# ilur98/DLMC-QUANT

Hardware: AMD Instinct MI355X
Metric: ResNet-50 W8A8 fake-quant fwd images/sec (higher is better)
Workload: dtype i8; 1 GPU; resnet50 W8A8 per-channel fake-quant forward (FSPTQ forms: W minmax_channel s8, A minmax_tensor u8), BN folded first as in FSPTQuant.py:67, fused int8 MFMA conv/linear, frozen execution plan (epilogue-fused ReLU / shortcut / next-layer codes; block end + next 1x1 as one launch; weight codes quantised once at plan build), 2 HIP streams per GPU, 224x224 relu(N(0,1)) pixels, batch 512 per GPU, scales; global_batch=512, parallelism=dp1 (batch-sharded replicas)

## Files before the change

dlmc-quant_amd/csrc/conv_pwr_i8.hip:

```cpp
#include "conv_i8_common.h"

namespace dlmcq {

struct PwrArgs {
  const int8_t* x;
  const int8_t* w;
  const float* s_w;
  const int32_t* wsum;
  const float* bias;
  const float* s_in;
  const float* zp_in;
  const float* residual;
  float* out;
  int f_rowb, f_chunk;
  int M, K, shift, nslice;
  int nblk;
  const int8_t* x2;
  const int8_t* w2;
  const float* s_w2;
  const int32_t* wsum2;
  const float* bias2;
  const float* s_in2;
  const float* zp_in2;
  int shift2, P, Q, H2, W2, stride2;
  FastDiv qdiv, pdiv;
};

constexpr int PWR_BN = 128;
constexpr int PWR_FROW = 36;

__device__ __forceinline__ void bload16s(f32x4& dst, int voff, const v4i& rsrc, int soff) {
  asm volatile("buffer_load_dwordx4 %0, %1, %2, %3 offen" DLMCQ_NT : "=v"(dst) : "v"(voff), "s"(rsrc), "s"(soff) : "memory");
}
__device__ __forceinline__ void bstore16s(const f32x4& v, int voff, const v4i& rsrc, int soff) {
  asm volatile("buffer_store_dwordx4 %0, %1, %2, %3 offen" DLMCQ_NT "\n\ts_nop 1" ::"v"(v), "v"(voff), "s"(rsrc), "s"(soff) : "memory");
}

template <int C, int NW, bool OUTF, bool CODES = true, int C2 = 0, bool SWP = false>
__global__ __launch_bounds__(NW * 64, NW / 4) void conv_pwr_i8_kernel(PwrArgs a, ConvEpi ep) {
  static_assert(OUTF || CODES, "nothing to produce");
  constexpr bool RES = C2 == 0;
  constexpr int NA2 = C2 / 32;
  constexpr int WB2 = C2 * PWR_BN;
  constexpr int NPAR = RES ? 3 : 6;
  constexpr int BN = PWR_BN;
  constexpr int S = C / 64;
  constexpr int NA = C / 32;
  constexpr int NP = BN / 32;
  constexpr int WB = C * BN;
  constexpr int PIECES = S * (BN / 16);
  constexpr int O = OUTF ? 4 : 0;
  constexpr int SROW = BN + 16;
  constexpr int NST = CODES ? 4 : 0;
  extern __shared__ __attribute__((aligned(1024))) int8_t pwr_lds[];
  int8_t* const wl = pwr_lds;
  int8_t* const wl2 = pwr_lds + WB;
  int8_t* const par = pwr_lds + WB + WB2;
  const int tid = threadIdx.x, wave = tid >> 6, lane = tid & 63, l31 = lane & 31, hsel = lane >> 5;
  int8_t* const stg = pwr_lds + WB + WB2 + NPAR * BN * 4 + wave * (32 * SROW + 32 * PWR_FROW * 4);
  float* const fst = reinterpret_cast<float*>(stg + 32 * SROW);
  const int rsel = lane >> 3, q4 = lane & 7;

  const uint32_t b = blockIdx.x;
  const int slice = (int)((b >> 3) % (uint32_t)a.nslice);
  const int group = (int)((b >> 3) / (uint32_t)a.nslice) * 8 + (int)(b & 7u);
  const int ngroups = (int)(gridDim.x / (uint32_t)a.nslice);
  const int n0 = slice * BN;

  {
    const void* arrs[6] = {a.s_w, a.wsum, a.bias, a.s_w2, a.wsum2, a.bias2};
#pragma unroll
    for (int r = 0; r < NPAR; ++r) {
      if (!arrs[r]) {
        for (int c = tid; c < BN; c += NW * 64) reinterpret_cast<float*>(par)[r * BN + c] = 0.0f;
        continue;
      }
      for (int c = wave; c < BN / 64; c += NW)
        __builtin_amdgcn_global_load_lds((gptr_t)(static_cast<const int32_t*>(arrs[r]) + n0 + c * 64 + lane), (lptr_t)(par + (r * BN + c * 64) * 4), 4, 0, 0);
    }
    const int lrow = lane >> 2, pslot = lane & 3;
    for (int pc = wave; pc < PIECES; pc += NW) {
      const int s = pc / (BN / 16), r16 = pc - s * (BN / 16);
      const int row = r16 * 16 + lrow;
      const int d = row & 31;
      const int k = n0 + (row & ~31) + 16 * ((d >> 2) & 1) + 4 * (d >> 3) + (d & 3);
      const int seg = pslot ^ ((row >> 2) & 3);
      __builtin_amdgcn_global_load_lds((gptr_t)(a.w + (int64_t)k * C + s * 64 + seg * 16), (lptr_t)(wl + s * (BN * 64) + r16 * 1024), 16, 0, 0);
    }
    for (int pc = wave; pc < (C2 / 64) * (BN / 16); pc += NW) {
      const int s = pc / (BN / 16), r16 = pc - s * (BN / 16);
      const int row = r16 * 16 + lrow;
      const int d = row & 31;
      const int k = n0 + (row & ~31) + 16 * ((d >> 2) & 1) + 4 * (d >> 3) + (d & 3);
      const int seg = pslot ^ ((row >> 2) & 3);
      __builtin_amdgcn_global_load_lds((gptr_t)(a.w2 + (int64_t)k * C2 + s * 64 + seg * 16), (lptr_t)(wl2 + s * (BN * 64) + r16 * 1024), 16, 0, 0);
    }
  }
  const float zpf = a.zp_in ? a.zp_in[0] : 0.0f;
  const int zpi = (int)__builtin_rintf(zpf);
  const float sin = a.s_in[0];
  const uint32_t xorw = a.shift ? 0x80808080u : 0u;
  const EpiQuant eq(ep, true);
  const v4i r_x = make_rsrc(a.x, (uint32_t)((int64_t)a.M * C));
  const v4i r_c = make_rsrc(CODES ? ep.codes : nullptr, CODES ? (uint32_t)((int64_t)a.M * a.K) : 0u);
  const v4i r_r = make_rsrc(RES ? a.residual : nullptr, RES ? (uint32_t)((int64_t)a.M * a.K * 4) : 0u);
  const v4i r_x2 = make_rsrc(RES ? nullptr : a.x2, RES ? 0u : (uint32_t)((int64_t)(a.M / (a.P * a.Q)) * a.H2 * a.W2 * C2));
  const uint32_t xorw2 = (!RES && a.shift2) ? 0x80808080u : 0u;
  const v4i r_o = make_rsrc(OUTF ? a.out : nullptr, OUTF ? (uint32_t)((int64_t)a.M * a.K * 4) : 0u);
  const int so8 = __builtin_amdgcn_readfirstlane(8 * a.f_rowb);
  const int fchunk = __builtin_amdgcn_readfirstlane(a.f_chunk);
  auto poff = [&](int p) { return (p >> 1) * fchunk + (p & 1) * 128; };

  i32x4 areg[NA];
  i32x4 areg2[RES ? 1 : NA2];
  f32x4 res[2][4];
  auto request = [&](int blk) {
    const int vo = blk < a.nblk ? (blk * 32 + l31) * C + hsel * 16 : BUF_BIG;
    static_for<NA>([&](auto f) { bload16i<decltype(f)::value * 32>(areg[decltype(f)::value], vo, r_x); });
    if constexpr (!RES) {
      const uint32_t m = (uint32_t)(blk * 32 + l31);
      const uint32_t t = fdiv(m, a.qdiv);
      const int q = (int)(m - t * (uint32_t)a.Q);
      const uint32_t n = fdiv(t, a.pdiv);
      const int pp = (int)(t - n * (uint32_t)a.P);
      const int vo2 = blk < a.nblk ? (((int)n * a.H2 + pp * a.stride2) * a.W2 + q * a.stride2) * C2 + hsel * 16 : BUF_BIG;
      static_for<NA2>([&](auto f) { bload16i<(decltype(f)::value % 64) * 32>(areg2[decltype(f)::value], vo2 + (decltype(f)::value / 64) * 2048, r_x2); });
    }
  };
  auto fbase = [&](int blk) { return blk < a.nblk ? (blk * 32 + rsel) * a.f_rowb + slice * 2 * fchunk + 16 * q4 : BUF_BIG; };
  const int stride = ngroups * NW;
  int blk = group * NW + wave;
  request(blk);
  if constexpr (RES) {
    const int vb = fbase(blk);
#pragma unroll
    for (int it = 0; it < 4; ++it) bload16s(res[0][it], vb, r_r, it * so8);
  }
  asm volatile("s_waitcnt vmcnt(0)" ::: "memory");
  __syncthreads();
  if (tid < BN) {
    float* pf = reinterpret_cast<float*>(par) + tid;
    int* pi = reinterpret_cast<int*>(par) + BN + tid;
    *pf = sin * *pf;
    *pi = (a.shift - zpi) * *pi;
    if constexpr (!RES) {
      const float zp2 = a.zp_in2 ? a.zp_in2[0] : 0.0f;
      pf[3 * BN] = a.s_in2[0] * pf[3 * BN];
      pi[3 * BN] = (a.shift2 - (int)__builtin_rintf(zp2)) * pi[3 * BN];
    }
  }
  __syncthreads();

  for (; blk < a.nblk; blk += stride) {
    asm volatile("s_waitcnt vmcnt(%0)" ::"n"(O + NST) : "memory");
#pragma unroll
    for (int f = 0; f < NA; ++f) {
      asm volatile("" : "+v"(areg[f]));
      areg[f] = i32x4{(int)(areg[f].x ^ xorw), (int)(areg[f].y ^ xorw), (int)(areg[f].z ^ xorw), (int)(areg[f].w ^ xorw)};
    }
    if constexpr (!RES) {
#pragma unroll
      for (int f = 0; f < NA2; ++f) {
        asm volatile("" : "+v"(areg2[f]));
        areg2[f] = i32x4{(int)(areg2[f].x ^ xorw2), (int)(areg2[f].y ^ xorw2), (int)(areg2[f].z ^ xorw2), (int)(areg2[f].w ^ xorw2)};
      }
    }
    const int vb = fbase(blk);
    const int vbn = fbase(blk + stride);
    static_for<NP>([&](auto p_c) {
      constexpr int p = decltype(p_c)::value;
      constexpr int cur = p & 1, nxt = cur ^ 1;
      if constexpr (RES) {
#pragma unroll
        for (int it = 0; it < 4; ++it) bload16s(res[nxt][it], (p + 1 < NP ? vb + poff(p + 1) : vbn), r_r, it * so8);
      }
      f32x2 ex[RES ? 1 : 8];
      if constexpr (!RES) {
        i32x16 acc2;
        const i32x4* cop = reinterpret_cast<const i32x4*>(par + (4 * BN + p * 32 + hsel * 16) * 4);
#pragma unroll
        for (int q = 0; q < 4; ++q) {
          const i32x4 c4 = cop[q];
          acc2[4 * q] = c4.x;
          acc2[4 * q + 1] = c4.y;
          acc2[4 * q + 2] = c4.z;
          acc2[4 * q + 3] = c4.w;
        }
        static_for<NA2>([&](auto f_c) {
          constexpr int f = decltype(f_c)::value;
          constexpr int s = f >> 1, ks = f & 1;
          const int sg = ks * 2 + hsel;
          const int brow = p * 32 + l31;
          const i32x4 bf = *reinterpret_cast<const i32x4*>(wl2 + s * (BN * 64) + brow * 64 + ((sg ^ ((brow >> 2) & 3)) << 4));
          acc2 = __builtin_amdgcn_mfma_i32_32x32x32_i8(bf, areg2[f], acc2, 0, 0, 0);
        });
        const int cb2 = p * 32 + hsel * 16;
#pragma unroll
        for (int q = 0; q < 4; ++q) {
          const f32x4 mu = *reinterpret_cast<const f32x4*>(par + (3 * BN + cb2 + 4 * q) * 4);
          const f32x4 bs = *reinterpret_cast<const f32x4*>(par + (5 * BN + cb2 + 4 * q) * 4);
          ex[RES ? 0 : 2 * q] = pk_fma(f32x2{(float)acc2[4 * q], (float)acc2[4 * q + 1]}, f32x2{mu.x, mu.y}, f32x2{bs.x, bs.y});
          ex[RES ? 0 : 2 * q + 1] = pk_fma(f32x2{(float)acc2[4 * q + 2], (float)acc2[4 * q + 3]}, f32x2{mu.z, mu.w}, f32x2{bs.z, bs.w});
        }
      }
      i32x16 acc;
      {
        const i32x4* cop = reinterpret_cast<const i32x4*>(par + (BN + p * 32 + hsel * 16) * 4);
#pragma unroll
        for (int q = 0; q < 4; ++q) {
          const i32x4 c4 = cop[q];
          acc[4 * q] = c4.x;
          acc[4 * q + 1] = c4.y;
          acc[4 * q + 2] = c4.z;
          acc[4 * q + 3] = c4.w;
        }
      }
      static_for<NA>([&](auto f_c) {
        constexpr int f = decltype(f_c)::value;
        constexpr int s = f >> 1, ks = f & 1;
        const int sg = ks * 2 + hsel;
        const int brow = p * 32 + l31;
        const i32x4 bf = *reinterpret_cast<const i32x4*>(wl + s * (BN * 64) + brow * 64 + ((sg ^ ((brow >> 2) & 3)) << 4));
        acc = __builtin_amdgcn_mfma_i32_32x32x32_i8(bf, areg[f], acc, 0, 0, 0);
      });
      if constexpr (p == NP - 1) request(blk + stride);
      const int cb = p * 32 + hsel * 16;
#pragma unroll
      for (int q = 0; q < 4; ++q) {
        const f32x4 mu = *reinterpret_cast<const f32x4*>(par + (cb + 4 * q) * 4);
        const f32x4 bs = *reinterpret_cast<const f32x4*>(par + (2 * BN + cb + 4 * q) * 4);
        f32x2 ya = pk_fma(f32x2{(float)acc[4 * q], (float)acc[4 * q + 1]}, f32x2{mu.x, mu.y}, f32x2{bs.x, bs.y});
        f32x2 yb = pk_fma(f32x2{(float)acc[4 * q + 2], (float)acc[4 * q + 3]}, f32x2{mu.z, mu.w}, f32x2{bs.z, bs.w});
        if constexpr (!RES) {
          ya = SWP ? ex[RES ? 0 : 2 * q] + ya : ya + ex[RES ? 0 : 2 * q];
          yb = SWP ? ex[RES ? 0 : 2 * q + 1] + yb : yb + ex[RES ? 0 : 2 * q + 1];
        }
        *reinterpret_cast<f32x4*>(fst + l31 * PWR_FROW + hsel * 16 + 4 * q) = f32x4{ya.x, ya.y, yb.x, yb.y};
      }
      asm volatile("s_waitcnt lgkmcnt(0)" ::: "memory");
      if constexpr (RES && p > 0) asm volatile("s_waitcnt vmcnt(%0)" ::"n"(O + 4 + (p == NP - 1 ? NA : 0)) : "memory");
      f32x4 v[4];
#pragma unroll
      for (int it = 0; it < 4; ++it) {
        const f32x4 y = *reinterpret_cast<const f32x4*>(fst + (it * 8 + rsel) * PWR_FROW + 4 * q4);
        if constexpr (RES) {
          asm volatile("" : "+v"(res[cur][it]));
          const f32x2 va = f32x2{y.x, y.y} + f32x2{res[cur][it].x, res[cur][it].y};
          const f32x2 vc = f32x2{y.z, y.w} + f32x2{res[cur][it].z, res[cur][it].w};
          v[it] = f32x4{va.x, va.y, vc.x, vc.y};
        } else {
          v[it] = y;
        }
        if constexpr (OUTF) {
          v[it] = relu4_nan(v[it]);
          bstore16s(v[it], vb + poff(p), r_o, it * so8);
        }
      }
      asm volatile("s_waitcnt lgkmcnt(0)" ::: "memory");
      if constexpr (CODES) {
        uint32_t wq[4];
        eq.code4n_plain(v, wq);
#pragma unroll
        for (int it = 0; it < 4; ++it) *reinterpret_cast<uint32_t*>(stg + (it * 8 + rsel) * SROW + p * 32 + 4 * q4) = wq[it];
      }
    });
    if constexpr (CODES) {
      const int vc = blk < a.nblk ? (blk * 32 + rsel) * a.K + n0 + q4 * 16 : BUF_BIG;
#pragma unroll
      for (int it = 0; it < NST; ++it) {
        const i32x4 c16 = *reinterpret_cast<const i32x4*>(stg + (it * 8 + rsel) * SROW + q4 * 16);
        asm volatile("buffer_store_dwordx4 %0, %1, %2, %3 offen\n\ts_nop 1" ::"v"(c16), "v"(vc), "s"(r_c), "s"(it * 8 * a.K) : "memory");
      }
    }
  }
  asm volatile("s_waitcnt vmcnt(0)" ::: "memory");
}

bool conv_pwr_applies(int64_t N, int64_t H, int64_t W, int64_t C, int64_t K, int64_t R, int64_t S, int32_t stride, int32_t pad,
                      int32_t dilation, const ConvEpi& ep, const float* out, const ConvSeg2* seg2) {
  if (R != 1 || S != 1 || pad != 0 || dilation != 1 || !ep.relu || ep.w_off) return false;
  if (ep.relu == DLMCQ_ACT_RELU6) return false;
  if (ep.codes ? !epi_plain(ep) : !out) return false;
  const int64_t P = (H - 1) / stride + 1, Q = (W - 1) / stride + 1;
  const int64_t M = N * P * Q;
  if (seg2) {
    const ConvGeom& g2 = seg2->g;
    if (ep.residual || !out || !ep.codes || g2.R != 1 || g2.S != 1 || g2.pad != 0 || g2.dil != 1 || g2.P != P || g2.Q != Q) return false;
    const bool main_dense = stride == 1 && C == 256 && g2.C == 512, seg_dense = g2.stride == 1 && g2.C == 256 && C == 512;
    if (!main_dense && !seg_dense) return false;
    if ((main_dense ? N * g2.H * g2.W : N * H * W) * 512 >= (int64_t)BUF_BIG) return false;
  } else {
    if (stride != 1 || !ep.residual || !(C == 256 || C == 512)) return false;
    if (M * C >= (int64_t)BUF_BIG) return false;
  }
  if (K % PWR_BN != 0 || K > 4096) return false;
  if (ep.residual && out && ((ep.ctl & DLMCQ_FP32_IN_CHUNK_MAJOR) != 0) != ((ep.ctl & DLMCQ_FP32_OUT_CHUNK_MAJOR) != 0)) return false;
  if ((ep.codes && !aligned16(ep.codes)) || (ep.residual && !aligned16(ep.residual)) || (out && !aligned16(out))) return false;
  if (M < 4096 || M % 32 != 0) return false;
  if (M * K * 4 >= (int64_t)BUF_BIG) return false;
  return true;
}

template <int C, int NW, bool OUTF, bool CODES = true, int C2 = 0, bool SWP = false>
static int pwr_go(const PwrArgs& a0, const ConvEpi& ep, hipStream_t st) {
  constexpr int LDS = (C + C2) * PWR_BN + (C2 ? 6 : 3) * PWR_BN * 4 + NW * (32 * (PWR_BN + 16) + 32 * PWR_FROW * 4);
  static_assert(LDS <= 160 * 1024, "LDS");
  PwrArgs a = a0;
  a.nslice = a.K / PWR_BN;
  static int cus = 0;
  if (!cus) {
    int dev = 0;
    hipDeviceProp_t prop;
    cus = (hipGetDevice(&dev) == hipSuccess && hipGetDeviceProperties(&prop, dev) == hipSuccess && prop.multiProcessorCount > 0)
              ? prop.multiProcessorCount : 256;
  }
  int ngroups = (cus / a.nslice) & ~7;
  if (ngroups < 8) ngroups = 8;
  const int maxg = ((a.nblk + NW - 1) / NW + 7) & ~7;
  if (ngroups > maxg) ngroups = maxg;
  auto kern = conv_pwr_i8_kernel<C, NW, OUTF, CODES, C2, SWP>;
  static bool attr_set = false;
  if (!attr_set) {
    const hipError_t e = hipFuncSetAttribute(reinterpret_cast<const void*>(kern), hipFuncAttributeMaxDynamicSharedMemorySize, LDS);
    if (e != hipSuccess) return (int)e;
    attr_set = true;
  }
  hipLaunchKernelGGL(kern, dim3((uint32_t)(ngroups * a.nslice)), dim3(NW * 64), LDS, st, a, ep);
  return launch_status();
}

int conv_pwr_launch(const int8_t* x, const int8_t* w, float* out, const float* bias, const int32_t* wsum, const float* in_scale,
                    const float* in_zero_point, const float* w_scale, int64_t N, int64_t H, int64_t W, int64_t C, int64_t K, int32_t stride,
                    int shift, const ConvEpi& ep, hipStream_t st, const ConvSeg2* seg2) {
  const int64_t P = (H - 1) / stride + 1, Q = (W - 1) / stride + 1;
  PwrArgs a{};
  a.x = x; a.w = w; a.s_w = w_scale; a.wsum = wsum; a.bias = bias; a.s_in = in_scale; a.zp_in = in_zero_point;
  a.residual = ep.residual; a.out = out;
  a.M = (int)(N * P * Q); a.K = (int)K; a.shift = shift;
  a.nblk = a.M / 32;
  const bool fcm = (ep.ctl & (ep.residual ? DLMCQ_FP32_IN_CHUNK_MAJOR : DLMCQ_FP32_OUT_CHUNK_MAJOR)) != 0;
  a.f_rowb = fcm ? 256 : a.K * 4;
  a.f_chunk = fcm ? a.M * 256 : 256;
#ifndef DLMCQ_PWR_NW256
#define DLMCQ_PWR_NW256 12
#endif
#ifndef DLMCQ_PWR_NW512
#define DLMCQ_PWR_NW512 8
#endif
  constexpr int N2 = DLMCQ_PWR_NW256, N5 = DLMCQ_PWR_NW512;
  if (seg2) {
    const ConvGeom& g2 = seg2->g;
    a.P = (int)P; a.Q = (int)Q;
    a.qdiv = make_fastdiv((uint32_t)Q);
    a.pdiv = make_fastdiv((uint32_t)P);
    if (C == 256) {
      a.x2 = seg2->x; a.w2 = seg2->w; a.s_w2 = seg2->s_w; a.wsum2 = seg2->wsum; a.bias2 = seg2->bias; a.s_in2 = seg2->s_in; a.zp_in2 = seg2->zp_in;
      a.shift2 = seg2->shift; a.H2 = g2.H; a.W2 = g2.W; a.stride2 = g2.stride;
      return pwr_go<256, 6, true, true, 512, false>(a, ep, st);
    }
    a.x = seg2->x; a.w = seg2->w; a.s_w = seg2->s_w; a.wsum = seg2->wsum; a.bias = seg2->bias; a.s_in = seg2->s_in; a.zp_in = seg2->zp_in;
    a.shift = seg2->shift;
    a.x2 = x; a.w2 = w; a.s_w2 = w_scale; a.wsum2 = wsum; a.bias2 = bias; a.s_in2 = in_scale; a.zp_in2 = in_zero_point;
    a.shift2 = shift; a.H2 = (int)H; a.W2 = (int)W; a.stride2 = stride;
    return pwr_go<256, 6, true, true, 512, true>(a, ep, st);
  }
  if (!ep.codes) return C == 256 ? pwr_go<256, N2, true, false>(a, ep, st) : (C == 512 ? pwr_go<512, N5, true, false>(a, ep, st) : DLMCQ_EINVAL);
  if (C == 256) return out ? pwr_go<256, N2, true>(a, ep, st) : pwr_go<256, N2, false>(a, ep, st);
  if (C == 512) return out ? pwr_go<512, N5, true>(a, ep, st) : pwr_go<512, N5, false>(a, ep, st);
  return DLMCQ_EINVAL;
}

}
```

Before: 93720 images/s.

## Extend dual-GEMM projection fusion to the 512/1024-channel stage with 64-wide slices

```diff
diff --git a/dlmc-quant_amd/csrc/conv_pwr_i8.hip b/dlmc-quant_amd/csrc/conv_pwr_i8.hip
--- a/dlmc-quant_amd/csrc/conv_pwr_i8.hip
+++ b/dlmc-quant_amd/csrc/conv_pwr_i8.hip
@@ -36,14 +36,16 @@
   asm volatile("buffer_store_dwordx4 %0, %1, %2, %3 offen" DLMCQ_NT "\n\ts_nop 1" ::"v"(v), "v"(voff), "s"(rsrc), "s"(soff) : "memory");
 }
 
-template <int C, int NW, bool OUTF, bool CODES = true, int C2 = 0, bool SWP = false>
+template <int C, int NW, bool OUTF, bool CODES = true, int C2 = 0, bool SWP = false, int BN = PWR_BN>
 __global__ __launch_bounds__(NW * 64, NW / 4) void conv_pwr_i8_kernel(PwrArgs a, ConvEpi ep) {
   static_assert(OUTF || CODES, "nothing to produce");
+  static_assert(BN == 64 || BN == 128, "slice width");
   constexpr bool RES = C2 == 0;
-  constexpr int NA2 = C2 / 32;
-  constexpr int WB2 = C2 * PWR_BN;
+  constexpr bool DEEP = C2 > 512;
+  static_assert(!DEEP || (BN == 64 && OUTF && CODES && C2 % 64 == 0), "the deep dual form: 64-wide slices, fp32 output and codes");
+  constexpr int NA2 = DEEP ? C2 / 64 : C2 / 32;
+  constexpr int WB2 = C2 * BN;
   constexpr int NPAR = RES ? 3 : 6;
-  constexpr int BN = PWR_BN;
   constexpr int S = C / 64;
   constexpr int NA = C / 32;
   constexpr int NP = BN / 32;
@@ -51,7 +53,9 @@
   constexpr int PIECES = S * (BN / 16);
   constexpr int O = OUTF ? 4 : 0;
   constexpr int SROW = BN + 16;
-  constexpr int NST = CODES ? 4 : 0;
+  constexpr int LPR = BN / 16;
+  constexpr int RPI = 64 / LPR;
+  constexpr int NST = CODES ? 32 / RPI : 0;
   extern __shared__ __attribute__((aligned(1024))) int8_t pwr_lds[];
   int8_t* const wl = pwr_lds;
   int8_t* const wl2 = pwr_lds + WB;
@@ -114,20 +118,36 @@
   i32x4 areg[NA];
   i32x4 areg2[RES ? 1 : NA2];
   f32x4 res[2][4];
-  auto request = [&](int blk) {
+  auto request_main = [&](int blk) {
     const int vo = blk < a.nblk ? (blk * 32 + l31) * C + hsel * 16 : BUF_BIG;
     static_for<NA>([&](auto f) { bload16i<decltype(f)::value * 32>(areg[decltype(f)::value], vo, r_x); });
-    if constexpr (!RES) {
-      const uint32_t m = (uint32_t)(blk * 32 + l31);
-      const uint32_t t = fdiv(m, a.qdiv);
-      const int q = (int)(m - t * (uint32_t)a.Q);
-      const uint32_t n = fdiv(t, a.pdiv);
-      const int pp = (int)(t - n * (uint32_t)a.P);
-      const int vo2 = blk < a.nblk ? (((int)n * a.H2 + pp * a.stride2) * a.W2 + q * a.stride2) * C2 + hsel * 16 : BUF_BIG;
-      static_for<NA2>([&](auto f) { bload16i<(decltype(f)::value % 64) * 32>(areg2[decltype(f)::value], vo2 + (decltype(f)::value / 64) * 2048, r_x2); });
-    }
   };
-  auto fbase = [&](int blk) { return blk < a.nblk ? (blk * 32 + rsel) * a.f_rowb + slice * 2 * fchunk + 16 * q4 : BUF_BIG; };
+  auto sampled_off = [&](int blk) {
+    const uint32_t m = (uint32_t)(blk * 32 + l31);
+    const uint32_t t = fdiv(m, a.qdiv);
+    const int q = (int)(m - t * (uint32_t)a.Q);
+    const uint32_t n = fdiv(t, a.pdiv);
+    const int pp = (int)(t - n * (uint32_t)a.P);
+    return blk < a.nblk ? (((int)n * a.H2 + pp * a.stride2) * a.W2 + q * a.stride2) * C2 + hsel * 16 : BUF_BIG;
+  };
+  auto request_sampled = [&](int vo2, auto half) {
+    constexpr int F0 = decltype(half)::value * NA2;
+    static_for<NA2>([&](auto f) { bload16i<((F0 + decltype(f)::value) % 64) * 32>(areg2[decltype(f)::value], vo2 + ((F0 + decltype(f)::value) / 64) * 2048, r_x2); });
+  };
+  auto request = [&](int blk) {
+    request_main(blk);
+    if constexpr (!RES) request_sampled(sampled_off(blk), std::integral_constant<int, 0>{});
+  };
+  auto fbase = [&](int blk) { return blk < a.nblk ? (blk * 32 + rsel) * a.f_rowb + slice * (BN / 64) * fchunk + 16 * q4 : BUF_BIG; };
+  auto store_codes = [&](int blk) {
+    const int crow = lane / LPR, cq = lane % LPR;
+    const int vc = blk < a.nblk ? (blk * 32 + crow) * a.K + n0 + cq * 16 : BUF_BIG;
+#pragma unroll
+    for (int it = 0; it < NST; ++it) {
+      const i32x4 c16 = *reinterpret_cast<const i32x4*>(stg + (it * RPI + crow) * SROW + cq * 16);
+      asm volatile("buffer_store_dwordx4 %0, %1, %2, %3 offen\n\ts_nop 1" ::"v"(c16), "v"(vc), "s"(r_c), "s"(it * RPI * a.K) : "memory");
+    }
+  };
   const int stride = ngroups * NW;
   int blk = group * NW + wave;
   request(blk);
@@ -151,6 +171,93 @@
   }
   __syncthreads();
 
+  if constexpr (DEEP) {
+  for (; blk < a.nblk; blk += stride) {
+    asm volatile("s_waitcnt vmcnt(%0)" ::"n"(O + NST) : "memory");
+    auto landed = [&](i32x4* r, auto n_c, uint32_t xw) {
+#pragma unroll
+      for (int f = 0; f < decltype(n_c)::value; ++f) {
+        asm volatile("" : "+v"(r[f]));
+        r[f] = i32x4{(int)(r[f].x ^ xw), (int)(r[f].y ^ xw), (int)(r[f].z ^ xw), (int)(r[f].w ^ xw)};
+      }
+    };
+    landed(areg, std::integral_constant<int, NA>{}, xorw);
+    landed(areg2, std::integral_constant<int, NA2>{}, xorw2);
+    i32x16 acc[NP], acc2[NP];
+    auto start = [&](i32x16& c, int row, int p) {
+      const i32x4* cop = reinterpret_cast<const i32x4*>(par + (row * BN + p * 32 + hsel * 16) * 4);
+#pragma unroll
+      for (int q = 0; q < 4; ++q) {
+        const i32x4 c4 = cop[q];
+        c[4 * q] = c4.x;
+        c[4 * q + 1] = c4.y;
+        c[4 * q + 2] = c4.z;
+        c[4 * q + 3] = c4.w;
+      }
+    };
+    auto wfrag = [&](const int8_t* wbase, int f, int p) {
+      const int s = f >> 1, sg = (f & 1) * 2 + hsel, brow = p * 32 + l31;
+      return *reinterpret_cast<const i32x4*>(wbase + s * (BN * 64) + brow * 64 + ((sg ^ ((brow >> 2) & 3)) << 4));
+    };
+    static_for<NP>([&](auto p_c) { start(acc2[decltype(p_c)::value], 4, decltype(p_c)::value); });
+    static_for<NA2>([&](auto f_c) {
+      static_for<NP>([&](auto p_c) {
+        constexpr int f = decltype(f_c)::value, p = decltype(p_c)::value;
+        acc2[p] = __builtin_amdgcn_mfma_i32_32x32x32_i8(wfrag(wl2, f, p), areg2[f], acc2[p], 0, 0, 0);
+      });
+    });
+    request_sampled(sampled_off(blk), std::integral_constant<int, 1>{});
+    static_for<NP>([&](auto p_c) { start(acc[decltype(p_c)::value], 1, decltype(p_c)::value); });
+    static_for<NA>([&](auto f_c) {
+      static_for<NP>([&](auto p_c) {
+        constexpr int f = decltype(f_c)::value, p = decltype(p_c)::value;
+        acc[p] = __builtin_amdgcn_mfma_i32_32x32x32_i8(wfrag(wl, f, p), areg[f], acc[p], 0, 0, 0);
+      });
+    });
+    request_main(blk + stride);
+    asm volatile("s_waitcnt vmcnt(%0)" ::"n"(NA) : "memory");
+    landed(areg2, std::integral_constant<int, NA2>{}, xorw2);
+    static_for<NA2>([&](auto f_c) {
+      static_for<NP>([&](auto p_c) {
+        constexpr int f = decltype(f_c)::value, p = decltype(p_c)::value;
+        acc2[p] = __builtin_amdgcn_mfma_i32_32x32x32_i8(wfrag(wl2, NA2 + f, p), areg2[f], acc2[p], 0, 0, 0);
+      });
+    });
+    const int vb = fbase(blk);
+    static_for<NP>([&](auto p_c) {
+      constexpr int p = decltype(p_c)::value;
+      const int cb = p * 32 + hsel * 16;
+#pragma unroll
+      for (int q = 0; q < 4; ++q) {
+        const f32x4 mu2 = *reinterpret_cast<const f32x4*>(par + (3 * BN + cb + 4 * q) * 4);
+        const f32x4 bs2 = *reinterpret_cast<const f32x4*>(par + (5 * BN + cb + 4 * q) * 4);
+        const f32x2 ea = pk_fma(f32x2{(float)acc2[p][4 * q], (float)acc2[p][4 * q + 1]}, f32x2{mu2.x, mu2.y}, f32x2{bs2.x, bs2.y});
+        const f32x2 eb = pk_fma(f32x2{(float)acc2[p][4 * q + 2], (float)acc2[p][4 * q + 3]}, f32x2{mu2.z, mu2.w}, f32x2{bs2.z, bs2.w});
+        const f32x4 mu = *reinterpret_cast<const f32x4*>(par + (cb + 4 * q) * 4);
+        const f32x4 bs = *reinterpret_cast<const f32x4*>(par + (2 * BN + cb + 4 * q) * 4);
+        f32x2 ya = pk_fma(f32x2{(float)acc[p][4 * q], (float)acc[p][4 * q + 1]}, f32x2{mu.x, mu.y}, f32x2{bs.x, bs.y});
+        f32x2 yb = pk_fma(f32x2{(float)acc[p][4 * q + 2], (float)acc[p][4 * q + 3]}, f32x2{mu.z, mu.w}, f32x2{bs.z, bs.w});
+        ya = SWP ? ea + ya : ya + ea;
+        yb = SWP ? eb + yb : yb + eb;
+        *reinterpret_cast<f32x4*>(fst + l31 * PWR_FROW + hsel * 16 + 4 * q) = f32x4{ya.x, ya.y, yb.x, yb.y};
+      }
+      asm volatile("s_waitcnt lgkmcnt(0)" ::: "memory");
+      f32x4 v[4];
+#pragma unroll
+      for (int it = 0; it < 4; ++it) {
+        v[it] = relu4_nan(*reinterpret_cast<const f32x4*>(fst + (it * 8 + rsel) * PWR_FROW + 4 * q4));
+        bstore16s(v[it], vb + poff(p), r_o, it * so8);
+      }
+      asm volatile("s_waitcnt lgkmcnt(0)" ::: "memory");
+      uint32_t wq[4];
+      eq.code4n_plain(v, wq);
+#pragma unroll
+      for (int it = 0; it < 4; ++it) *reinterpret_cast<uint32_t*>(stg + (it * 8 + rsel) * SROW + p * 32 + 4 * q4) = wq[it];
+      if constexpr (p == 0) request_sampled(sampled_off(blk + stride), std::integral_constant<int, 0>{});
+    });
+    store_codes(blk);
+  }
+  } else {
   for (; blk < a.nblk; blk += stride) {
     asm volatile("s_waitcnt vmcnt(%0)" ::"n"(O + NST) : "memory");
 #pragma unroll
@@ -264,14 +371,8 @@
         for (int it = 0; it < 4; ++it) *reinterpret_cast<uint32_t*>(stg + (it * 8 + rsel) * SROW + p * 32 + 4 * q4) = wq[it];
       }
     });
-    if constexpr (CODES) {
-      const int vc = blk < a.nblk ? (blk * 32 + rsel) * a.K + n0 + q4 * 16 : BUF_BIG;
-#pragma unroll
-      for (int it = 0; it < NST; ++it) {
-        const i32x4 c16 = *reinterpret_cast<const i32x4*>(stg + (it * 8 + rsel) * SROW + q4 * 16);
-        asm volatile("buffer_store_dwordx4 %0, %1, %2, %3 offen\n\ts_nop 1" ::"v"(c16), "v"(vc), "s"(r_c), "s"(it * 8 * a.K) : "memory");
-      }
-    }
+    if constexpr (CODES) store_codes(blk);
+  }
   }
   asm volatile("s_waitcnt vmcnt(0)" ::: "memory");
 }
@@ -286,9 +387,10 @@
   if (seg2) {
     const ConvGeom& g2 = seg2->g;
     if (ep.residual || !out || !ep.codes || g2.R != 1 || g2.S != 1 || g2.pad != 0 || g2.dil != 1 || g2.P != P || g2.Q != Q) return false;
-    const bool main_dense = stride == 1 && C == 256 && g2.C == 512, seg_dense = g2.stride == 1 && g2.C == 256 && C == 512;
+    auto pair = [](int64_t cd, int64_t cs) { return (cd == 256 && cs == 512) || (cd == 512 && cs == 1024); };
+    const bool main_dense = stride == 1 && pair(C, g2.C), seg_dense = g2.stride == 1 && pair(g2.C, C);
     if (!main_dense && !seg_dense) return false;
-    if ((main_dense ? N * g2.H * g2.W : N * H * W) * 512 >= (int64_t)BUF_BIG) return false;
+    if ((main_dense ? N * g2.H * g2.W * g2.C : N * H * W * C) >= (int64_t)BUF_BIG) return false;
   } else {
     if (stride != 1 || !ep.residual || !(C == 256 || C == 512)) return false;
     if (M * C >= (int64_t)BUF_BIG) return false;
@@ -301,24 +403,18 @@
   return true;
 }
 
-template <int C, int NW, bool OUTF, bool CODES = true, int C2 = 0, bool SWP = false>
+template <int C, int NW, bool OUTF, bool CODES = true, int C2 = 0, bool SWP = false, int BN = PWR_BN>
 static int pwr_go(const PwrArgs& a0, const ConvEpi& ep, hipStream_t st) {
-  constexpr int LDS = (C + C2) * PWR_BN + (C2 ? 6 : 3) * PWR_BN * 4 + NW * (32 * (PWR_BN + 16) + 32 * PWR_FROW * 4);
+  constexpr int LDS = (C + C2) * BN + (C2 ? 6 : 3) * BN * 4 + NW * (32 * (BN + 16) + 32 * PWR_FROW * 4);
   static_assert(LDS <= 160 * 1024, "LDS");
   PwrArgs a = a0;
-  a.nslice = a.K / PWR_BN;
-  static int cus = 0;
-  if (!cus) {
-    int dev = 0;
-    hipDeviceProp_t prop;
-    cus = (hipGetDevice(&dev) == hipSuccess && hipGetDeviceProperties(&prop, dev) == hipSuccess && prop.multiProcessorCount > 0)
-              ? prop.multiProcessorCount : 256;
-  }
+  a.nslice = a.K / BN;
+  const int cus = device_cus();
   int ngroups = (cus / a.nslice) & ~7;
   if (ngroups < 8) ngroups = 8;
   const int maxg = ((a.nblk + NW - 1) / NW + 7) & ~7;
   if (ngroups > maxg) ngroups = maxg;
-  auto kern = conv_pwr_i8_kernel<C, NW, OUTF, CODES, C2, SWP>;
+  auto kern = conv_pwr_i8_kernel<C, NW, OUTF, CODES, C2, SWP, BN>;
   static bool attr_set = false;
   if (!attr_set) {
     const hipError_t e = hipFuncSetAttribute(reinterpret_cast<const void*>(kern), hipFuncAttributeMaxDynamicSharedMemorySize, LDS);
@@ -347,22 +443,26 @@
 #ifndef DLMCQ_PWR_NW512
 #define DLMCQ_PWR_NW512 8
 #endif
-  constexpr int N2 = DLMCQ_PWR_NW256, N5 = DLMCQ_PWR_NW512;
+#ifndef DLMCQ_PWR_NWDEEP
+#define DLMCQ_PWR_NWDEEP 8
+#endif
+  constexpr int N2 = DLMCQ_PWR_NW256, N5 = DLMCQ_PWR_NW512, NWD = DLMCQ_PWR_NWDEEP;
   if (seg2) {
     const ConvGeom& g2 = seg2->g;
     a.P = (int)P; a.Q = (int)Q;
     a.qdiv = make_fastdiv((uint32_t)Q);
     a.pdiv = make_fastdiv((uint32_t)P);
-    if (C == 256) {
+    const bool deep = C + g2.C == 1536;
+    if (C == 256 || (deep && C == 512)) {
       a.x2 = seg2->x; a.w2 = seg2->w; a.s_w2 = seg2->s_w; a.wsum2 = seg2->wsum; a.bias2 = seg2->bias; a.s_in2 = seg2->s_in; a.zp_in2 = seg2->zp_in;
       a.shift2 = seg2->shift; a.H2 = g2.H; a.W2 = g2.W; a.stride2 = g2.stride;
-      return pwr_go<256, 6, true, true, 512, false>(a, ep, st);
+      return deep ? pwr_go<512, NWD, true, true, 1024, false, 64>(a, ep, st) : pwr_go<256, 6, true, true, 512, false>(a, ep, st);
     }
     a.x = seg2->x; a.w = seg2->w; a.s_w = seg2->s_w; a.wsum = seg2->wsum; a.bias = seg2->bias; a.s_in = seg2->s_in; a.zp_in = seg2->zp_in;
     a.shift = seg2->shift;
     a.x2 = x; a.w2 = w; a.s_w2 = w_scale; a.wsum2 = wsum; a.bias2 = bias; a.s_in2 = in_scale; a.zp_in2 = in_zero_point;
     a.shift2 = shift; a.H2 = (int)H; a.W2 = (int)W; a.stride2 = stride;
-    return pwr_go<256, 6, true, true, 512, true>(a, ep, st);
+    return deep ? pwr_go<512, NWD, true, true, 1024, true, 64>(a, ep, st) : pwr_go<256, 6, true, true, 512, true>(a, ep, st);
   }
   if (!ep.codes) return C == 256 ? pwr_go<256, N2, true, false>(a, ep, st) : (C == 512 ? pwr_go<512, N5, true, false>(a, ep, st) : DLMCQ_EINVAL);
   if (C == 256) return out ? pwr_go<256, N2, true>(a, ep, st) : pwr_go<256, N2, false>(a, ep, st);
```

Result: no change. 92950 images/s (-0.8%).
